# ylongqi/openrec

Hardware: AMD Instinct MI355X
Metric: BPR training triplets/sec at dim=64, 1Mx1M table (higher is better)
Workload: dtype f32; 1 GPU; bpr dim=64 1000000x1000000 table, batch=65536 triplets/GPU, sgd lr=0.05, objective loss+l2_loss, exact TF duplicate semantics; parallelism=single-gpu

## Files before the change

openrec_amd/csrc/kernels_plan.hip:

```cpp
#include "orx_internal.h"

#include "orx_device.h"

#include <cstring>
#include <vector>
#include <algorithm>

constexpr int PL_THREADS = 256;
constexpr int PL_REFS = 8;
constexpr int PL_CHUNK = PL_THREADS * PL_REFS;
constexpr int PL_LCNT = 1024;

struct PlanArgs {
    DedupArgs d;
    int shift;
    int nru, nri;
    int lgu, lgi;
    int* bcnt;
    int2* list;
    int64_t nref;
    unsigned int* dupbits;
    int min_late;
    int s_first;
    unsigned long long* tstamp;
};
#define PL_STAMP(i) do { if (a.tstamp != nullptr && threadIdx.x == 0) a.tstamp[((size_t)blockIdx.y * gridDim.x + blockIdx.x) * 8 + (i)] = wall_clock64(); } while (0)

__device__ __forceinline__ bool plan_ref(const PlanArgs& a, int64_t s, int64_t j, int& id, bool& is_user, int& pos) {
    const DedupArgs& d = a.d;
    if (j < d.nU) { id = d.uid[s * d.id_stride + j]; is_user = true; pos = (int)j; }
    else if (j < d.nU + d.nP) { id = d.pid[s * d.id_stride + (j - d.nU)]; is_user = false; pos = (int)(d.role_stride ? d.role_stride + (j - d.nU) : j); }
    else { id = d.nid[s * d.id_stride + (j - d.nU - d.nP)]; is_user = false; pos = (int)(d.role_stride ? 2 * d.role_stride + (j - d.nU - d.nP) : j); }
    return id_ok(id, is_user ? d.NU : d.NI);
}

__device__ __forceinline__ int32_t* plan_idword(const DedupArgs& d, int64_t s, int pos) {
    if (d.pair_tpw > 1) {
        const int Bp = (int)d.role_stride;
        const int slot = (pos >= Bp ? 1 : 0) + (pos >= 2 * Bp ? 1 : 0);
        return reinterpret_cast<int32_t*>(d.ids4 + s * d.pair_stride + (pos - slot * Bp)) + slot;
    }
    return d.ids_out + s * d.flag_stride + pos;
}

__device__ __forceinline__ void pl_lds_barrier() { asm volatile("s_waitcnt lgkmcnt(0)\n\ts_barrier" ::: "memory"); }

template <int T = PL_THREADS>
__device__ __forceinline__ int plan_scan_excl(int v, int* wave_tot, int& total) {
    const int lane = threadIdx.x & 63, wave = threadIdx.x >> 6;
    int incl = v;
#pragma unroll
    for (int o = 1; o < 64; o <<= 1) { const int t = __shfl_up(incl, o); if (lane >= o) incl += t; }
    if (lane == 63) wave_tot[wave] = incl;
    pl_lds_barrier();
    int before = 0, all = 0;
#pragma unroll
    for (int k = 0; k < T / 64; ++k) { const int t = wave_tot[k]; if (k < wave) before += t; all += t; }
    pl_lds_barrier();
    total = all;
    return before + incl - v;
}

template <bool SCATTER>
__global__ __launch_bounds__(PL_THREADS) void plan_part_kernel(PlanArgs a) {
    extern __shared__ int pl_hist[];
    const int nb = a.nru + a.nri;
    const int64_t s = blockIdx.y;
    int* hist = pl_hist;
    int* base = pl_hist + nb;
    for (int i = threadIdx.x; i < nb; i += PL_THREADS) hist[i] = 0;
    __syncthreads();
    const int64_t j0 = (int64_t)blockIdx.x * PL_CHUNK + threadIdx.x;
    int bk[PL_REFS], rk[PL_REFS], idv[PL_REFS], posv[PL_REFS];
#pragma unroll
    for (int k = 0; k < PL_REFS; ++k) {
        const int64_t j = j0 + (int64_t)k * PL_THREADS;
        bk[k] = -1;
        if (j < a.nref) {
            int id, pos; bool is_user;
            const bool ok = plan_ref(a, s, j, id, is_user, pos);
            if (ok) {
                bk[k] = is_user ? (id & (a.nru - 1)) : a.nru + (id & (a.nri - 1));
                idv[k] = id; posv[k] = pos;
            }
            if (SCATTER) {
                if (a.d.pair_tpw > 1) {
                    if (j < a.d.pair_stride) {
                        const int p = a.d.pid[s * a.d.id_stride + j];
                        const int n = a.d.label ? __float_as_int(a.d.label[s * a.d.id_stride + j]) : a.d.nid[s * a.d.id_stride + j];
                        const bool okp = id_ok(p, a.d.NI), okn = a.d.label ? true : id_ok(n, a.d.NI);
                        a.d.ids4[s * a.d.pair_stride + j] = make_int4(ok ? id : 0x7fffffff, okp ? p : 0x7fffffff, okn ? n : 0x7fffffff, (int)((uint32_t)j << 10));
                        if (!(ok & okp & okn)) {
                            const int poison = (int)(ORX_PARTNER_POISON | ((uint32_t)a.d.pair_gen << 24));
                            a.d.partner[s * a.d.pair_stride + j] = make_int4(poison, poison, poison, 0);
                        }
                    }
                } else {
                    a.d.ids_out[s * a.d.flag_stride + pos] = ok ? id : 0x7fffffff;
                }
            }
        }
    }
#pragma unroll
    for (int k = 0; k < PL_REFS; ++k) if (bk[k] >= 0) rk[k] = atomicAdd(&hist[bk[k]], 1);
    __syncthreads();
    int* cnt = a.bcnt + s * (3 * nb + 1);
    if (!SCATTER) {
        if (blockIdx.x == 0 && threadIdx.x < 8) a.d.alloc[8 * s + threadIdx.x] = 0;
        if (blockIdx.x == 0 && threadIdx.x == 8) a.d.dcount[s] = 0;
        for (int i = threadIdx.x; i < nb; i += PL_THREADS) { const int c = hist[i]; if (c) atomicAdd(cnt + i, c); }
        return;
    }
    __shared__ int wave_tot[PL_THREADS / 64];
    int* off = pl_hist + 2 * nb;
    for (int i = threadIdx.x; i < nb; i += PL_THREADS) off[i] = cnt[i];
    __syncthreads();
    {
        const int per = (nb + PL_THREADS - 1) / PL_THREADS;
        const int i0 = threadIdx.x * per;
        int mine = 0;
        for (int i = i0; i < i0 + per && i < nb; ++i) mine += off[i];
        int total;
        int run = plan_scan_excl(mine, wave_tot, total);
        for (int i = i0; i < i0 + per && i < nb; ++i) { const int c = off[i]; off[i] = run; run += c; }
        if (threadIdx.x == 0) off[nb] = total;
    }
    __syncthreads();
    if (blockIdx.x == 0) for (int i = threadIdx.x; i <= nb; i += PL_THREADS) cnt[2 * nb + i] = off[i];
    int* cur = cnt + nb;
    for (int i = threadIdx.x; i < nb; i += PL_THREADS) { const int c = hist[i]; if (c) base[i] = off[i] + atomicAdd(cur + i, c); }
    __syncthreads();
    int2* list = a.list + s * a.nref;
#pragma unroll
    for (int k = 0; k < PL_REFS; ++k) if (bk[k] >= 0) list[base[bk[k]] + rk[k]] = make_int2(idv[k], posv[k]);
}

__device__ __forceinline__ int pl_cnt(const int* p) { return __hip_atomic_load(p, __ATOMIC_RELAXED, __HIP_MEMORY_SCOPE_AGENT); }
__device__ __forceinline__ unsigned int pl_peek(const unsigned int* p) { return *reinterpret_cast<const volatile unsigned int*>(p); }

constexpr int PL_UN = 8;
template <int T, class F>
__device__ __forceinline__ void pl_for_each(const int2* ent, int n, F f) {
    for (int i0 = threadIdx.x; i0 < n; i0 += PL_UN * T) {
        int2 e[PL_UN];
#pragma unroll
        for (int k = 0; k < PL_UN; ++k) { const int i = i0 + k * T; if (i < n) e[k] = ent[i]; }
#pragma unroll
        for (int k = 0; k < PL_UN; ++k) { const int i = i0 + k * T; if (i < n) f(i, e[k]); }
    }
}

__device__ __forceinline__ int pl_rank(int* cnt, int dn) {
    const int lane = threadIdx.x & 63;
    int rank = -1;
    for (int round = 0; round < 4; ++round) {
        const unsigned long long todo = __ballot(rank < 0);
        if (!todo) break;
        const int ld = __shfl(dn, __ffsll((long long)todo) - 1);
        const bool mine = rank < 0 && dn == ld;
        const unsigned long long grp = __ballot(mine);
        const int gsz = __popcll(grp);
        if (gsz < 4) break;
        const int first = __ffsll((long long)grp) - 1;
        int base = 0;
        if (lane == first) base = atomicAdd(cnt + ld, gsz);
        base = __shfl(base, first);
        if (mine) rank = base + __popcll(grp & ((1ull << lane) - 1ull));
    }
    if (rank < 0) rank = atomicAdd(cnt + dn, 1);
    return rank;
}

constexpr int PL_PAIR_CAP = 512;

template <int T>
__global__ __launch_bounds__(T) void plan_range_kernel(PlanArgs a) {
    extern __shared__ __attribute__((aligned(16))) unsigned int pl_lds[];
    const DedupArgs& d = a.d;
    const int W = (1 << a.shift) >> 5;
    unsigned int* seen = pl_lds;
    unsigned int* dup = pl_lds + W;
    unsigned int* tri = pl_lds + 2 * W;
    unsigned short* prefix16 = reinterpret_cast<unsigned short*>(pl_lds + 3 * W);
    int* lcnt = reinterpret_cast<int*>(pl_lds + 3 * W + (W + 1) / 2);
    unsigned short* dprefix16 = reinterpret_cast<unsigned short*>(seen);
    int* pairpos = reinterpret_cast<int*>(lcnt + PL_LCNT);
    __shared__ int wave_tot[T / 64];
    __shared__ int sh_late, sh_dense, sh_seg, list_cnt, list_base;
    const int nb = a.nru + a.nri;
    const int b = blockIdx.x;
    const int64_t s = blockIdx.y;
    const bool is_user = b < a.nru;
    const int lg = is_user ? a.lgu : a.lgi;
    const int bl = is_user ? b : b - a.nru;
    const int* cnt = a.bcnt + s * (3 * nb + 1) + 2 * nb;
    PL_STAMP(0);
    if (b == 0) for (int i = threadIdx.x; i < 2 * nb; i += T) a.bcnt[s * (3 * nb + 1) + i] = 0;
    const int lo = cnt[b], n = cnt[b + 1] - lo;
    int2* ent = a.list + s * a.nref + lo;
    unsigned int* dupout = a.dupbits ? a.dupbits + ((size_t)s * nb + b) * W : nullptr;
    if (threadIdx.x == 0 && n > 8192) atomicMax(d.alloc + 8 * s + 6, n);
    if (n == 0) {
        if (dupout) for (int w = threadIdx.x; w < W; w += T) dupout[w] = 0u;
        return;
    }
    int2* refinfo = d.refinfo ? d.refinfo + s * d.flag_stride : nullptr;
    const bool small = n <= PL_UN * T;
    int2 er[PL_UN];
    if (small) {
#pragma unroll
        for (int k = 0; k < PL_UN; ++k) { const int i = threadIdx.x + k * T; if (i < n) er[k] = ent[i]; }
    }
    for (int i = threadIdx.x; i < 3 * W; i += T) pl_lds[i] = 0u;
    if (threadIdx.x == 0) { sh_late = 0; list_cnt = 0; }
    pl_lds_barrier();
    PL_STAMP(1);
    int late = 0;
    auto pass1 = [&](int2 e) -> int {
        const int l = e.x >> lg;
        const unsigned int bit = 1u << (l & 31);
        const unsigned int cur = pl_peek(&seen[l >> 5]);
        const unsigned int old = (cur & bit) ? cur : atomicOr(&seen[l >> 5], bit);
        int role = 0;
        if (old & bit) {
            const unsigned int cur2 = pl_peek(&dup[l >> 5]);
            const unsigned int old2 = (cur2 & bit) ? cur2 : atomicOr(&dup[l >> 5], bit);
            role = 1;
            if (old2 & bit) {
                if (!(pl_peek(&tri[l >> 5]) & bit)) atomicOr(&tri[l >> 5], bit);
                role = 2; ++late;
            }
        }
        return role;
    };
    if (small) {
#pragma unroll
        for (int k = 0; k < PL_UN; ++k) {
            const int i = threadIdx.x + k * T;
            if (i < n) er[k].y = (int)((uint32_t)er[k].y | ((uint32_t)pass1(er[k]) << 30));
        }
    } else {
        pl_for_each<T>(ent, n, [&](int i, int2 e) {
            const int role = pass1(e);
            if (role) ent[i].y = (int)((uint32_t)e.y | ((uint32_t)role << 30));
        });
    }
    if (late) atomicAdd(&sh_late, late);
    pl_lds_barrier();
    PL_STAMP(2);
    int mine = 0;
    for (int w = threadIdx.x; w < W; w += T) mine += __popc(dup[w]);
    int off = 0;
    if (mine) off = atomicAdd(&list_cnt, mine);
    pl_lds_barrier();
    int list_base_r = 0;
    if (threadIdx.x == 0 && list_cnt) {
        list_base_r = atomicAdd(d.dcount + s, list_cnt);
        atomicAdd(d.alloc + 8 * s + 5, list_cnt);
    }
    const bool want_plan = sh_late >= (a.min_late < 0 ? (n / 512 > 64 ? n / 512 : 64) : a.min_late);
    const bool plan = refinfo != nullptr && want_plan;
    if (want_plan && refinfo == nullptr && threadIdx.x == 0) atomicAdd(d.alloc + 8 * s + 1, sh_late);
    int ntri = 0, dense0 = 0;
    int* segstart = nullptr;
    if (plan) {
        segstart = d.segstart + s * d.tri_stride;
        const int per = (W + T - 1) / T;
        const int w0 = threadIdx.x * per;
        int mine3 = 0;
        for (int w = w0; w < w0 + per && w < W; ++w) mine3 += __popc(tri[w]);
        int pre = plan_scan_excl<T>(mine3, wave_tot, ntri);
        if (ntri > 65535) ntri = 0;
        if (ntri) {
            if (threadIdx.x == 0) sh_dense = atomicAdd(d.alloc + 8 * s, ntri);
            for (int w = w0; w < w0 + per && w < W; ++w) { prefix16[w] = (unsigned short)pre; pre += __popc(tri[w]); }
            __syncthreads();
            dense0 = sh_dense;
            if (ntri > PL_LCNT) lcnt = d.tricnt + s * d.tri_stride + dense0;
            for (int i = threadIdx.x; i < ntri; i += T) lcnt[i] = 0;
            __syncthreads();
        }
    }
    int ndup2 = 0;
    const bool pairing = d.pair_tpw > 1 && W <= 4096;
    if (pairing) {
        const int per = (W + T - 1) / T;
        const int w0 = threadIdx.x * per;
        int mine2 = 0;
        for (int w = w0; w < w0 + per && w < W; ++w) mine2 += __popc(dup[w] & ~tri[w]);
        int pre = plan_scan_excl<T>(mine2, wave_tot, ndup2);
        if (ndup2 > PL_PAIR_CAP) ndup2 = 0;
        if (ndup2) {
            for (int w = w0; w < w0 + per && w < W; ++w) { dprefix16[w] = (unsigned short)pre; pre += __popc(dup[w] & ~tri[w]); }
            for (int i = threadIdx.x; i < 2 * ndup2; i += T) pairpos[i] = -1;
            pl_lds_barrier();
        }
    }
    PL_STAMP(3);
    auto pass2 = [&](int2 e) {
        const int l = e.x >> lg;
        const int pos = e.y & 0x3fffffff;
        const unsigned int dw = dup[l >> 5];
        const unsigned int dd = (dw >> (l & 31)) & 1u;
        if (dd) {
            uint32_t v = (uint32_t)e.x | (1u << 31);
            const unsigned int tw = tri[l >> 5];
            const unsigned int t3 = (tw >> (l & 31)) & 1u;
            if (ndup2 && !t3) {
                const int dn2 = (int)dprefix16[l >> 5] + __popc(dw & ~tw & ((1u << (l & 31)) - 1u));
                pairpos[2 * dn2 + (int)(((uint32_t)e.y >> 30) & 1u)] = pos;
                return;
            }
            v |= (t3 ? 2u : ((uint32_t)e.y >> 30)) << 29;
            if (t3 && ntri) {
                const int dn = (int)prefix16[l >> 5] + __popc(tw & ((1u << (l & 31)) - 1u));
                refinfo[pos] = make_int2(dense0 + dn, pl_rank(lcnt, dn));
            } else if (t3 && refinfo != nullptr) {
                refinfo[pos] = make_int2(-1, 0);
            }
            *plan_idword(d, s, pos) = (int32_t)v;
        }
    };
    if (small) {
#pragma unroll
        for (int k = 0; k < PL_UN; ++k) { const int i = threadIdx.x + k * T; if (i < n) pass2(er[k]); }
    } else {
        pl_for_each<T>(ent, n, [&](int, int2 e) { pass2(e); });
    }
    PL_STAMP(4);
    if (ndup2) {
        pl_lds_barrier();
        int* partner = reinterpret_cast<int*>(d.partner + s * d.pair_stride);
        const int Bp = (int)d.role_stride;
        for (int k = threadIdx.x; k < ndup2; k += T) {
            const int posA = pairpos[2 * k], posB = pairpos[2 * k + 1];
            const int sa = (posA >= Bp ? 1 : 0) + (posA >= 2 * Bp ? 1 : 0), sb = (posB >= Bp ? 1 : 0) + (posB >= 2 * Bp ? 1 : 0);
            const int tag = d.pair_gen << 24;
            partner[4 * (posA - sa * Bp) + sa] = posB | tag;
            partner[4 * (posB - sb * Bp) + sb] = posA | (1 << 30) | tag;
        }
    }
    PL_STAMP(5);
    if (dupout) for (int w = threadIdx.x; w < W; w += T) dupout[w] = ndup2 ? tri[w] : dup[w];
    if (ntri) {
        __syncthreads();
        const int per = (ntri + T - 1) / T;
        const int d0 = threadIdx.x * per;
        int csum = 0;
        for (int k = d0; k < d0 + per && k < ntri; ++k) csum += pl_cnt(lcnt + k);
        int total_refs;
        int run = plan_scan_excl<T>(csum, wave_tot, total_refs);
        if (threadIdx.x == 0) sh_seg = atomicAdd(d.alloc + 8 * s + 1, total_refs);
        __syncthreads();
        run += sh_seg;
        for (int k = d0; k < d0 + per && k < ntri; ++k) { segstart[dense0 + k] = run; run += pl_cnt(lcnt + k); }
        __syncthreads();
    }
    PL_STAMP(6);
    if (threadIdx.x == 0) list_base = list_base_r;
    pl_lds_barrier();
    PL_STAMP(7);
    if (mine) {
        int64_t e = s * d.list_stride + list_base + off;
        const uint32_t tag = is_user ? 0u : 0x80000000u;
        for (int w = threadIdx.x; w < W; w += T) {
            unsigned int m = dup[w];
            const unsigned int m0 = m;
            const unsigned int tw = tri[w];
            while (m) {
                const int bpos = __ffs(m) - 1;
                m &= m - 1;
                if (ndup2 && !((tw >> bpos) & 1u)) {
                    const int dn2 = (int)dprefix16[w] + __popc(m0 & ~tw & ((1u << bpos) - 1u));
                    reinterpret_cast<int2*>(d.pslot)[e] = make_int2(pairpos[2 * dn2], pairpos[2 * dn2 + 1]);
                    if (d.dcnt != nullptr) { d.dseg[e] = 0; d.dcnt[e] = 0; }
                    ++e;
                    continue;
                }
                if (d.pair_tpw > 1) reinterpret_cast<int2*>(d.pslot)[e] = make_int2(-1, -1);
                d.dlist[e] = (uint32_t)((((int64_t)w * 32 + bpos) << lg) | bl) | tag;
                if (d.dcnt != nullptr) {
                    int c = 0, sg = 0;
                    if (ntri && ((tw >> bpos) & 1u)) {
                        const int dn = (int)prefix16[w] + __popc(tw & ((1u << bpos) - 1u));
                        c = pl_cnt(lcnt + dn);
                        sg = __hip_atomic_load(segstart + dense0 + dn, __ATOMIC_RELAXED, __HIP_MEMORY_SCOPE_AGENT);
                        if (c > ORX_SEG_DIRECT) {
                            int4* items = d.items + s * d.item_stride;
                            int src = sg, len = c, level = 0;
                            do {
                                const int pieces = (len + ORX_PIECE - 1) / ORX_PIECE;
                                const int b0 = d.tree_off[level] + atomicAdd(d.alloc + 8 * s + 2 + level, pieces);
                                for (int k = 0; k < pieces; ++k) {
                                    const int rem = len - k * ORX_PIECE;
                                    items[b0 + k] = make_int4(src + k * ORX_PIECE, rem < ORX_PIECE ? rem : ORX_PIECE, b0 + k, 0);
                                }
                                src = b0; len = pieces; ++level;
                            } while (len > ORX_SEG_DIRECT && level < 3);
                            sg = src; c = -len;
                        }
                    }
                    d.dseg[e] = sg; d.dcnt[e] = c;
                }
                ++e;
            }
        }
    }
}

template <int T>
__global__ __launch_bounds__(T) void plan_urgent_kernel(PlanArgs a) {
    extern __shared__ __attribute__((aligned(16))) unsigned int pl_lds[];
    const int W = (1 << a.shift) >> 5;
    const int nb = a.nru + a.nri;
    const int b = blockIdx.x;
    const int64_t s = a.s_first + blockIdx.y;
    const int* cnt = a.bcnt + s * (3 * nb + 1) + 2 * nb;
    const int lo = cnt[b], n = cnt[b + 1] - lo;
    if (n == 0) return;
    const int prev_n = cnt[b + 1 - (3 * nb + 1)] - cnt[b - (3 * nb + 1)];
    if (prev_n < 2) return;
    const unsigned int* prev = a.dupbits + ((s - 1) * nb + b) * (int64_t)W;
    for (int w = threadIdx.x; w < W; w += T) pl_lds[w] = prev[w];
    __syncthreads();
    const int lg = b < a.nru ? a.lgu : a.lgi;
    const int2* ent = a.list + s * a.nref + lo;
    pl_for_each<T>(ent, n, [&](int, int2 e) {
        const int l = e.x >> lg;
        if ((pl_lds[l >> 5] >> (l & 31)) & 1u) *plan_idword(a.d, s, e.y & 0x3fffffff) |= (1 << 28);
    });
}

__global__ __launch_bounds__(256) void plan_pair_kernel(PlanArgs a) {
    const DedupArgs& d = a.d;
    const int64_t s = blockIdx.y;
    const int B = (int)d.pair_stride, Bp = (int)d.role_stride, tpw = d.pair_tpw;
    const int4* part = d.partner + s * d.pair_stride;
    int* pword = reinterpret_cast<int*>(d.ids4 + s * d.pair_stride) + 3;
    const int nb = a.nru + a.nri, W = (1 << a.shift) >> 5;
    const int n = d.dcount[s];
    auto slot_of = [&](int pos) { return (pos >= Bp ? 1 : 0) + (pos >= 2 * Bp ? 1 : 0); };
    const uint32_t gen = (uint32_t)d.pair_gen;
    auto live = [gen](int w) { return (((uint32_t)w >> 24) & 63u) == gen && ((uint32_t)w & ORX_PARTNER_POS) != ORX_PARTNER_POISON; };
    auto poisoned = [gen](int4 r) {
        auto p = [gen](int w) { return (((uint32_t)w >> 24) & 63u) == gen && ((uint32_t)w & ORX_PARTNER_POS) == ORX_PARTNER_POISON; };
        return p(r.x) | p(r.y) | p(r.z);
    };
    auto choice = [live](int4 r) { return live(r.x) ? 0 : (live(r.y) ? 1 : (live(r.z) ? 2 : -1)); };
    auto word = [](int4 r, int k) { return k == 0 ? r.x : (k == 1 ? r.y : r.z); };
    const int4 none = make_int4(0, 0, 0, 0);
    int npair = 0;
    for (int e = blockIdx.x * 256 + threadIdx.x; e < n; e += gridDim.x * 256) {
        const int64_t eg = s * d.list_stride + e;
        const int2 ab = reinterpret_cast<const int2*>(d.pslot)[eg];
        const int posA = ab.x, posB = ab.y;
        if (posA < 0) continue;
        const int sa = slot_of(posA), sb = slot_of(posB);
        const int ta = posA - sa * Bp, tb = posB - sb * Bp;
        const int lo = ta < tb ? ta : tb, hi = ta < tb ? tb : ta;
        const int bl = lo ^ 1, bh = hi ^ 1;
        const bool same = (lo & ~(tpw - 1)) == (hi & ~(tpw - 1));
        const bool needq = ta != tb && !same;
        const int4 ra = part[ta], rb = part[tb];
        const int4 rl = (needq && bl < B) ? part[bl] : none, rh = (needq && bh < B) ? part[bh] : none;
        const bool mutual = (ta != tb) & (choice(ra) == sa) & (choice(rb) == sb) & !(poisoned(ra) | poisoned(rb));
        const int cl = choice(rl), ch = choice(rh);
        const int ppl = (int)((uint32_t)word(rl, cl) & ORX_PARTNER_POS), pph = (int)((uint32_t)word(rh, ch) & ORX_PARTNER_POS);
        const int syl = slot_of(ppl), syh = slot_of(pph);
        const int yl = ppl - syl * Bp, yh = pph - syh * Bp;
        const int4 ryl = (cl >= 0 && yl != bl) ? part[yl] : none, ryh = (ch >= 0 && yh != bh) ? part[yh] : none;
        const bool lo_taken = bl >= B || (cl >= 0 && yl != bl && choice(ryl) == syl);
        const bool hi_taken = bh >= B || (ch >= 0 && yh != bh && choice(ryh) == syh);
        bool acc = false;
        int stay = 0, mover = 0, q = 0;
        if (mutual) {
            if (same) { acc = true; stay = lo; mover = hi; q = hi; }
            else if (!lo_taken) { acc = true; stay = lo; mover = hi; q = bl; }
            else if (!hi_taken) { acc = true; stay = hi; mover = lo; q = bh; }
        }
        if (acc) {
            d.dlist[eg] = ORX_DLIST_DEAD;
            const uint32_t s_stay = (uint32_t)(stay == ta ? sa : sb), s_mov = (uint32_t)(stay == ta ? sb : sa), m = (uint32_t)tpw - 1u;
            pword[4 * stay] = (int)(ORX_PAIR_VALID | ORX_PAIR_WRITER | ((uint32_t)q & m) | (s_stay << 4) | (s_mov << 6) | ((uint32_t)stay << 10));
            pword[4 * q] = (int)(ORX_PAIR_VALID | ((uint32_t)stay & m) | (s_mov << 4) | (s_stay << 6) | ((uint32_t)mover << 10));
            if (q != mover) pword[4 * mover] = (int)((uint32_t)q << 10);
            reinterpret_cast<int2*>(d.pslot)[eg] = q != mover ? make_int2(q, mover) : make_int2(-1, -1);
            npair += 1;
        } else {
            reinterpret_cast<int2*>(d.pslot)[eg] = make_int2(-1, -1);
            int32_t* wa = plan_idword(d, s, posA);
            const uint32_t id = (uint32_t)*wa;
            *wa = (int32_t)(id | (1u << 31));
            *plan_idword(d, s, posB) = (int32_t)(id | (1u << 31) | (1u << 29));
            d.dlist[eg] = id | (sa ? 0x80000000u : 0u);
            if (a.dupbits != nullptr) {
                const int bk = sa ? a.nru + (int)(id & (uint32_t)(a.nri - 1)) : (int)(id & (uint32_t)(a.nru - 1));
                const int l = (int)(id >> (sa ? a.lgi : a.lgu));
                atomicOr(a.dupbits + ((size_t)s * nb + bk) * W + (l >> 5), 1u << (l & 31));
            }
        }
    }
    __shared__ int sh_np;
    if (threadIdx.x == 0) sh_np = 0;
    __syncthreads();
    if (npair) atomicAdd(&sh_np, npair);
    __syncthreads();
    if (threadIdx.x == 0 && sh_np) atomicAdd(d.alloc + 8 * s + 7, sh_np);
}

__global__ __launch_bounds__(256) void plan_swap_kernel(DedupArgs d) {
    const int64_t s = blockIdx.y;
    const int n = d.dcount[s];
    int4* rec = d.ids4 + s * d.pair_stride;
    for (int e = blockIdx.x * 256 + threadIdx.x; e < n; e += gridDim.x * 256) {
        const int2 qm = reinterpret_cast<const int2*>(d.pslot)[s * d.list_stride + e];
        if (qm.x < 0 || qm.y < 0) continue;
        const int4 a = rec[qm.x], b = rec[qm.y];
        rec[qm.x] = make_int4(b.x, b.y, b.z, a.w);
        rec[qm.y] = make_int4(a.x, a.y, a.z, b.w);
    }
}

int orx_launch_plan_swap(orx_ctx* ctx, const DedupArgs& d, int64_t kc) {
    if (d.pair_tpw < 2 || kc <= 0) return ORX_OK;
    ProfScope ps(ctx, ORX_K_DEDUP);
    ORX_LAUNCH(ctx, plan_swap_kernel, dim3((unsigned)std::max<int64_t>(4, (d.pair_stride / 4 + 255) / 256), (unsigned)kc), dim3(256), 0, d);
    ORX_HIP(hipGetLastError());
    return ORX_OK;
}

static int plan_buckets(int64_t rows, int64_t nref_t) {
    if (rows <= 0 || nref_t <= 0) return 0;
    const int cap = rows > (1LL << 27) ? 18 : 17;
    int64_t want = std::max<int64_t>((rows + (1LL << cap) - 1) >> cap, std::min<int64_t>(nref_t / 2048, rows / 64));
    static const char* env = getenv("ORX_PLAN_SHIFT");
    if (env) want = std::max<int64_t>(want, (rows + (1LL << atoi(env)) - 1) >> atoi(env));
    int n = 1;
    while (n < want && n < 8192) n *= 2;
    return n;
}
static int ilog2(int64_t n) { int l = 0; while ((1LL << l) < n) ++l; return l; }
static void plan_geometry(const DedupArgs& d, PlanArgs* a) {
    a->nref = d.nU + d.nP + d.nN;
    a->nru = plan_buckets(d.nU ? d.NU : 0, d.nU);
    a->nri = plan_buckets((d.nP + d.nN) ? d.NI : 0, d.nP + d.nN);
    a->lgu = ilog2(a->nru > 0 ? a->nru : 1); a->lgi = ilog2(a->nri > 0 ? a->nri : 1);
    const int64_t per_u = a->nru ? (d.NU + a->nru - 1) / a->nru : 1, per_i = a->nri ? (d.NI + a->nri - 1) / a->nri : 1;
    a->shift = std::max(5, ilog2(std::max(per_u, per_i)));
}

void orx_plan_geometry_query(const DedupArgs& d, int32_t out[14]) {
    PlanArgs a;
    plan_geometry(d, &a);
    out[0] = a.nru; out[1] = a.nri; out[2] = a.lgu; out[3] = a.lgi; out[4] = a.shift; out[5] = (1 << a.shift) >> 5;
    out[6] = PL_UN; out[7] = PL_LCNT; out[8] = PL_PAIR_CAP; out[9] = ORX_SEG_DIRECT; out[10] = ORX_PIECE;
    out[11] = PL_THREADS; out[12] = 1024; out[13] = PL_CHUNK;
}

static int plan_ensure(orx_ctx* c, int64_t chunk, const PlanArgs& a, bool want_dupbits) {
    const int nb = a.nru + a.nri;
    if (orx_ensure((void**)&c->d_pl_cnt, &c->d_pl_cnt_cap, (size_t)chunk * (3 * nb + 1) * sizeof(int))) return ORX_ERR_OOM;
    if (orx_ensure((void**)&c->d_pl_list, &c->d_pl_list_cap, (size_t)chunk * a.nref * sizeof(int2))) return ORX_ERR_OOM;
    const size_t words = (size_t)nb * ((1u << a.shift) >> 5);
    if (want_dupbits && orx_ensure((void**)&c->d_dupbits, &c->d_dupbits_cap, (size_t)chunk * words * sizeof(unsigned int))) return ORX_ERR_OOM;
    return ORX_OK;
}

int orx_plan_buffers(orx_ctx* c, int64_t chunk, int64_t B, int64_t NU, int64_t NI, bool want_dupbits) {
    const int64_t shapes[3][3] = {{B, B, B}, {B, B, 0}, {0, B, 0}};
    for (const auto& sh : shapes) {
        DedupArgs d;
        memset(&d, 0, sizeof(d));
        d.nU = sh[0]; d.nP = sh[1]; d.nN = sh[2]; d.NU = NU; d.NI = NI;
        PlanArgs a;
        plan_geometry(d, &a);
        const int rc = plan_ensure(c, chunk, a, want_dupbits);
        if (rc != ORX_OK) return rc;
    }
    return ORX_OK;
}

int orx_launch_plan(orx_ctx* ctx, const DedupArgs& d, int64_t kc, bool keep_dupbits, int64_t step0) {
    ProfScope ps(ctx, ORX_K_DEDUP);
    PlanArgs a;
    a.d = d;
    plan_geometry(d, &a);
    const int nb = a.nru + a.nri;
    if (nb == 0 || a.nref == 0 || kc == 0) return ORX_OK;
    ORX_ARG(a.nref < (1LL << 30) && kc < 65536, "plan: too many references per step (%lld) or steps (%lld)", (long long)a.nref, (long long)kc);
    { const int rc = plan_ensure(ctx, step0 + kc, a, keep_dupbits); if (rc != ORX_OK) return rc; }
    const size_t words = (size_t)nb * ((1u << a.shift) >> 5);
    a.bcnt = ctx->d_pl_cnt + step0 * (3 * nb + 1); a.list = ctx->d_pl_list + step0 * a.nref;
    a.dupbits = keep_dupbits ? ctx->d_dupbits + step0 * words : nullptr;
    a.s_first = 1;
    a.tstamp = nullptr;
    static const bool timing = getenv("ORX_PLAN_TIMING") != nullptr;
    if (timing) {
        ORX_HIP(hipMalloc((void**)&a.tstamp, (size_t)nb * kc * 8 * sizeof(unsigned long long)));
        ORX_HIP(hipMemsetAsync(a.tstamp, 0, (size_t)nb * kc * 8 * sizeof(unsigned long long), ctx->stream));
    }
    const char* ml = getenv("ORX_PLAN_MIN_LATE");
    a.min_late = ml ? atoi(ml) : d.min_late;
    if (ctx->pl_cnt_clean != ctx->d_pl_cnt || ctx->pl_cnt_clean_cap != ctx->d_pl_cnt_cap || ctx->pl_cnt_nb != nb)
        ORX_HIP(hipMemsetAsync(ctx->d_pl_cnt, 0, ctx->d_pl_cnt_cap, ctx->stream));
    ctx->pl_cnt_clean = nullptr;
    struct CleanMark { orx_ctx* c; int nb; bool ok = false;
                       ~CleanMark() { if (ok) { c->pl_cnt_clean = c->d_pl_cnt; c->pl_cnt_clean_cap = c->d_pl_cnt_cap; c->pl_cnt_nb = nb; } } } clean_mark{ctx, nb};
    const dim3 gp((unsigned)((a.nref + PL_CHUNK - 1) / PL_CHUNK), (unsigned)kc);
    const size_t hist_bytes = (size_t)(3 * nb + 1) * sizeof(int);
    ORX_ONCE_PER_DEVICE(ctx, ORX_HIP(hipFuncSetAttribute((const void*)plan_part_kernel<false>, hipFuncAttributeMaxDynamicSharedMemorySize, 128 * 1024)));
    ORX_ONCE_PER_DEVICE(ctx, ORX_HIP(hipFuncSetAttribute((const void*)plan_part_kernel<true>, hipFuncAttributeMaxDynamicSharedMemorySize, 128 * 1024)));
    ORX_ONCE_PER_DEVICE(ctx, ORX_HIP(hipFuncSetAttribute((const void*)plan_range_kernel<256>, hipFuncAttributeMaxDynamicSharedMemorySize, 140 * 1024)));
    ORX_ONCE_PER_DEVICE(ctx, ORX_HIP(hipFuncSetAttribute((const void*)plan_range_kernel<1024>, hipFuncAttributeMaxDynamicSharedMemorySize, 140 * 1024)));
    ORX_LAUNCH(ctx, (plan_part_kernel<false>), gp, dim3(PL_THREADS), hist_bytes, a);
    ORX_LAUNCH(ctx, (plan_part_kernel<true>), gp, dim3(PL_THREADS), hist_bytes, a);
    const int W = (1 << a.shift) >> 5;
    const size_t lds = (size_t)(3 * W + (W + 1) / 2) * 4 + (size_t)PL_LCNT * 4 +
                       (d.pair_tpw > 1 && W <= 4096 ? (size_t)2 * PL_PAIR_CAP * 4 : 0);
    if (ctx->plan_big) ORX_LAUNCH(ctx, plan_range_kernel<1024>, dim3((unsigned)nb, (unsigned)kc), dim3(1024), lds, a);
    else ORX_LAUNCH(ctx, plan_range_kernel<256>, dim3((unsigned)nb, (unsigned)kc), dim3(256), lds, a);
    if (d.pair_tpw > 1) ORX_LAUNCH(ctx, plan_pair_kernel, dim3((unsigned)std::max<int64_t>(4, (d.pair_stride / 4 + 255) / 256), (unsigned)kc), dim3(256), 0, a);
    ORX_HIP(hipGetLastError());
    clean_mark.ok = true;
    if (a.tstamp != nullptr) {
        ORX_HIP(hipStreamSynchronize(ctx->stream));
        std::vector<unsigned long long> h((size_t)nb * kc * 8);
        ORX_HIP(hipMemcpy(h.data(), a.tstamp, h.size() * sizeof(unsigned long long), hipMemcpyDeviceToHost));
        ORX_HIP(hipFree(a.tstamp));
        double sum[8] = {0}; unsigned long long t_min = ~0ull, t_max = 0; size_t live = 0;
        for (size_t w = 0; w < (size_t)nb * kc; ++w) {
            const unsigned long long* t = &h[w * 8];
            if (t[7] == 0) continue;
            ++live; t_min = std::min(t_min, t[0]); t_max = std::max(t_max, t[7]);
            for (int i = 1; i < 8; ++i) sum[i] += (double)(t[i] - t[i - 1]);
        }
        fprintf(stderr, "[orx plan timing] K=%lld, %zu workgroups, span %.1f us; mean us per phase: zero+cnt %.2f | pass1 %.2f | staging+prefix %.2f | pass2 %.2f | "
                "pairing %.2f | dupbits %.2f | list alloc %.2f\n", (long long)kc, live, (double)(t_max - t_min) * 0.01,
                sum[1] / live * 0.01, sum[2] / live * 0.01, sum[3] / live * 0.01, sum[4] / live * 0.01, sum[5] / live * 0.01, sum[6] / live * 0.01, sum[7] / live * 0.01);
    }
    return ORX_OK;
}

int orx_launch_plan_urgent(orx_ctx* ctx, const DedupArgs& d, int64_t kc, int64_t step0) {
    ProfScope ps(ctx, ORX_K_DEDUP);
    const int first = step0 > 0 ? 0 : 1;
    if (kc - first < 1) return ORX_OK;
    PlanArgs a;
    a.d = d;
    plan_geometry(d, &a);
    const int nb = a.nru + a.nri;
    const size_t words = (size_t)nb * ((1u << a.shift) >> 5);
    a.bcnt = ctx->d_pl_cnt + step0 * (3 * nb + 1); a.list = ctx->d_pl_list + step0 * a.nref; a.dupbits = ctx->d_dupbits + step0 * words; a.min_late = -1;
    a.s_first = first;
    a.tstamp = nullptr;
    const int W = (1 << a.shift) >> 5;
    if (ctx->plan_big) ORX_LAUNCH(ctx, plan_urgent_kernel<1024>, dim3((unsigned)(a.nru + a.nri), (unsigned)(kc - first)), dim3(1024), (size_t)W * 4, a);
    else ORX_LAUNCH(ctx, plan_urgent_kernel<256>, dim3((unsigned)(a.nru + a.nri), (unsigned)(kc - first)), dim3(256), (size_t)W * 4, a);
    ORX_HIP(hipGetLastError());
    return ORX_OK;
}
```

Baseline: 2.097 billion triplets/s.

## Flatten plan kernel grids and map each step's workgroups to one XCD

Replaces the 2D (block, step) launch grids of the plan kernels with a 1D grid. A remap function decodes each linear workgroup id so that all workgroups of a given step land on the same XCD under round-robin dispatch across the 8 XCDs. Per-step histogram atomics and count/list traffic then stay within one XCD's L2 instead of bouncing between XCDs. It adds index arithmetic per workgroup and depends on the hardware dispatching workgroups round-robin over XCDs.

```diff
diff --git a/openrec_amd/csrc/kernels_plan.hip b/openrec_amd/csrc/kernels_plan.hip
--- a/openrec_amd/csrc/kernels_plan.hip
+++ b/openrec_amd/csrc/kernels_plan.hip
@@ -1,6 +1,7 @@
 #include "orx_internal.h"
 
 #include "orx_device.h"
+#include "orx_plan_order.h"
 
 #include <cstring>
 #include <vector>
@@ -23,8 +24,10 @@
     int min_late;
     int s_first;
     unsigned long long* tstamp;
+    int gx, kc;
 };
-#define PL_STAMP(i) do { if (a.tstamp != nullptr && threadIdx.x == 0) a.tstamp[((size_t)blockIdx.y * gridDim.x + blockIdx.x) * 8 + (i)] = wall_clock64(); } while (0)
+#define PL_STAMP(i) do { if (a.tstamp != nullptr && threadIdx.x == 0) a.tstamp[((size_t)s * a.gx + b) * 8 + (i)] = wall_clock64(); } while (0)
+#define PL_WG(gx, kc) const OrxPlanWg pl_wg = orx_plan_order(blockIdx.x, (gx), (kc))
 
 __device__ __forceinline__ bool plan_ref(const PlanArgs& a, int64_t s, int64_t j, int& id, bool& is_user, int& pos) {
     const DedupArgs& d = a.d;
@@ -65,12 +68,14 @@
 __global__ __launch_bounds__(PL_THREADS) void plan_part_kernel(PlanArgs a) {
     extern __shared__ int pl_hist[];
     const int nb = a.nru + a.nri;
-    const int64_t s = blockIdx.y;
+    PL_WG(a.gx, a.kc);
+    const int64_t s = pl_wg.step;
+    const int blk = pl_wg.block;
     int* hist = pl_hist;
     int* base = pl_hist + nb;
     for (int i = threadIdx.x; i < nb; i += PL_THREADS) hist[i] = 0;
     __syncthreads();
-    const int64_t j0 = (int64_t)blockIdx.x * PL_CHUNK + threadIdx.x;
+    const int64_t j0 = (int64_t)blk * PL_CHUNK + threadIdx.x;
     int bk[PL_REFS], rk[PL_REFS], idv[PL_REFS], posv[PL_REFS];
 #pragma unroll
     for (int k = 0; k < PL_REFS; ++k) {
@@ -106,8 +111,8 @@
     __syncthreads();
     int* cnt = a.bcnt + s * (3 * nb + 1);
     if (!SCATTER) {
-        if (blockIdx.x == 0 && threadIdx.x < 8) a.d.alloc[8 * s + threadIdx.x] = 0;
-        if (blockIdx.x == 0 && threadIdx.x == 8) a.d.dcount[s] = 0;
+        if (blk == 0 && threadIdx.x < 8) a.d.alloc[8 * s + threadIdx.x] = 0;
+        if (blk == 0 && threadIdx.x == 8) a.d.dcount[s] = 0;
         for (int i = threadIdx.x; i < nb; i += PL_THREADS) { const int c = hist[i]; if (c) atomicAdd(cnt + i, c); }
         return;
     }
@@ -126,7 +131,7 @@
         if (threadIdx.x == 0) off[nb] = total;
     }
     __syncthreads();
-    if (blockIdx.x == 0) for (int i = threadIdx.x; i <= nb; i += PL_THREADS) cnt[2 * nb + i] = off[i];
+    if (blk == 0) for (int i = threadIdx.x; i <= nb; i += PL_THREADS) cnt[2 * nb + i] = off[i];
     int* cur = cnt + nb;
     for (int i = threadIdx.x; i < nb; i += PL_THREADS) { const int c = hist[i]; if (c) base[i] = off[i] + atomicAdd(cur + i, c); }
     __syncthreads();
@@ -188,8 +193,9 @@
     __shared__ int wave_tot[T / 64];
     __shared__ int sh_late, sh_dense, sh_seg, list_cnt, list_base;
     const int nb = a.nru + a.nri;
-    const int b = blockIdx.x;
-    const int64_t s = blockIdx.y;
+    PL_WG(a.gx, a.kc);
+    const int b = pl_wg.block;
+    const int64_t s = pl_wg.step;
     const bool is_user = b < a.nru;
     const int lg = is_user ? a.lgu : a.lgi;
     const int bl = is_user ? b : b - a.nru;
@@ -413,8 +419,9 @@
     extern __shared__ __attribute__((aligned(16))) unsigned int pl_lds[];
     const int W = (1 << a.shift) >> 5;
     const int nb = a.nru + a.nri;
-    const int b = blockIdx.x;
-    const int64_t s = a.s_first + blockIdx.y;
+    PL_WG(a.gx, a.kc);
+    const int b = pl_wg.block;
+    const int64_t s = a.s_first + pl_wg.step;
     const int* cnt = a.bcnt + s * (3 * nb + 1) + 2 * nb;
     const int lo = cnt[b], n = cnt[b + 1] - lo;
     if (n == 0) return;
@@ -433,7 +440,8 @@
 
 __global__ __launch_bounds__(256) void plan_pair_kernel(PlanArgs a) {
     const DedupArgs& d = a.d;
-    const int64_t s = blockIdx.y;
+    PL_WG(a.gx, a.kc);
+    const int64_t s = pl_wg.step;
     const int B = (int)d.pair_stride, Bp = (int)d.role_stride, tpw = d.pair_tpw;
     const int4* part = d.partner + s * d.pair_stride;
     int* pword = reinterpret_cast<int*>(d.ids4 + s * d.pair_stride) + 3;
@@ -450,7 +458,7 @@
     auto word = [](int4 r, int k) { return k == 0 ? r.x : (k == 1 ? r.y : r.z); };
     const int4 none = make_int4(0, 0, 0, 0);
     int npair = 0;
-    for (int e = blockIdx.x * 256 + threadIdx.x; e < n; e += gridDim.x * 256) {
+    for (int e = pl_wg.block * 256 + threadIdx.x; e < n; e += a.gx * 256) {
         const int64_t eg = s * d.list_stride + e;
         const int2 ab = reinterpret_cast<const int2*>(d.pslot)[eg];
         const int posA = ab.x, posB = ab.y;
@@ -508,11 +516,12 @@
     if (threadIdx.x == 0 && sh_np) atomicAdd(d.alloc + 8 * s + 7, sh_np);
 }
 
-__global__ __launch_bounds__(256) void plan_swap_kernel(DedupArgs d) {
-    const int64_t s = blockIdx.y;
+__global__ __launch_bounds__(256) void plan_swap_kernel(DedupArgs d, int gx, int kc) {
+    PL_WG(gx, kc);
+    const int64_t s = pl_wg.step;
     const int n = d.dcount[s];
     int4* rec = d.ids4 + s * d.pair_stride;
-    for (int e = blockIdx.x * 256 + threadIdx.x; e < n; e += gridDim.x * 256) {
+    for (int e = pl_wg.block * 256 + threadIdx.x; e < n; e += gx * 256) {
         const int2 qm = reinterpret_cast<const int2*>(d.pslot)[s * d.list_stride + e];
         if (qm.x < 0 || qm.y < 0) continue;
         const int4 a = rec[qm.x], b = rec[qm.y];
@@ -521,10 +530,15 @@
     }
 }
 
+static dim3 pl_grid(int64_t gx, int64_t kc) { return dim3((unsigned)(gx * kc)); }
+#define PL_GRID_OK(gx, kc) ORX_ARG((int64_t)(gx) * (int64_t)(kc) < (1LL << 31), "plan: %lld workgroups per step x %lld steps exceed a grid", (long long)(gx), (long long)(kc))
+
 int orx_launch_plan_swap(orx_ctx* ctx, const DedupArgs& d, int64_t kc) {
     if (d.pair_tpw < 2 || kc <= 0) return ORX_OK;
     ProfScope ps(ctx, ORX_K_DEDUP);
-    ORX_LAUNCH(ctx, plan_swap_kernel, dim3((unsigned)std::max<int64_t>(4, (d.pair_stride / 4 + 255) / 256), (unsigned)kc), dim3(256), 0, d);
+    const int gx = (int)std::max<int64_t>(4, (d.pair_stride / 4 + 255) / 256);
+    PL_GRID_OK(gx, kc);
+    ORX_LAUNCH(ctx, plan_swap_kernel, pl_grid(gx, kc), dim3(256), 0, d, gx, (int)kc);
     ORX_HIP(hipGetLastError());
     return ORX_OK;
 }
@@ -606,7 +620,10 @@
     ctx->pl_cnt_clean = nullptr;
     struct CleanMark { orx_ctx* c; int nb; bool ok = false;
                        ~CleanMark() { if (ok) { c->pl_cnt_clean = c->d_pl_cnt; c->pl_cnt_clean_cap = c->d_pl_cnt_cap; c->pl_cnt_nb = nb; } } } clean_mark{ctx, nb};
-    const dim3 gp((unsigned)((a.nref + PL_CHUNK - 1) / PL_CHUNK), (unsigned)kc);
+    a.kc = (int)kc;
+    a.gx = (int)((a.nref + PL_CHUNK - 1) / PL_CHUNK);
+    PL_GRID_OK(std::max<int64_t>(std::max(a.gx, nb), d.pair_stride / 1024 + 4), kc);
+    const dim3 gp = pl_grid(a.gx, kc);
     const size_t hist_bytes = (size_t)(3 * nb + 1) * sizeof(int);
     ORX_ONCE_PER_DEVICE(ctx, ORX_HIP(hipFuncSetAttribute((const void*)plan_part_kernel<false>, hipFuncAttributeMaxDynamicSharedMemorySize, 128 * 1024)));
     ORX_ONCE_PER_DEVICE(ctx, ORX_HIP(hipFuncSetAttribute((const void*)plan_part_kernel<true>, hipFuncAttributeMaxDynamicSharedMemorySize, 128 * 1024)));
@@ -617,9 +634,13 @@
     const int W = (1 << a.shift) >> 5;
     const size_t lds = (size_t)(3 * W + (W + 1) / 2) * 4 + (size_t)PL_LCNT * 4 +
                        (d.pair_tpw > 1 && W <= 4096 ? (size_t)2 * PL_PAIR_CAP * 4 : 0);
-    if (ctx->plan_big) ORX_LAUNCH(ctx, plan_range_kernel<1024>, dim3((unsigned)nb, (unsigned)kc), dim3(1024), lds, a);
-    else ORX_LAUNCH(ctx, plan_range_kernel<256>, dim3((unsigned)nb, (unsigned)kc), dim3(256), lds, a);
-    if (d.pair_tpw > 1) ORX_LAUNCH(ctx, plan_pair_kernel, dim3((unsigned)std::max<int64_t>(4, (d.pair_stride / 4 + 255) / 256), (unsigned)kc), dim3(256), 0, a);
+    a.gx = nb;
+    if (ctx->plan_big) ORX_LAUNCH(ctx, plan_range_kernel<1024>, pl_grid(nb, kc), dim3(1024), lds, a);
+    else ORX_LAUNCH(ctx, plan_range_kernel<256>, pl_grid(nb, kc), dim3(256), lds, a);
+    if (d.pair_tpw > 1) {
+        a.gx = (int)std::max<int64_t>(4, (d.pair_stride / 4 + 255) / 256);
+        ORX_LAUNCH(ctx, plan_pair_kernel, pl_grid(a.gx, kc), dim3(256), 0, a);
+    }
     ORX_HIP(hipGetLastError());
     clean_mark.ok = true;
     if (a.tstamp != nullptr) {
@@ -654,8 +675,10 @@
     a.s_first = first;
     a.tstamp = nullptr;
     const int W = (1 << a.shift) >> 5;
-    if (ctx->plan_big) ORX_LAUNCH(ctx, plan_urgent_kernel<1024>, dim3((unsigned)(a.nru + a.nri), (unsigned)(kc - first)), dim3(1024), (size_t)W * 4, a);
-    else ORX_LAUNCH(ctx, plan_urgent_kernel<256>, dim3((unsigned)(a.nru + a.nri), (unsigned)(kc - first)), dim3(256), (size_t)W * 4, a);
+    a.gx = nb; a.kc = (int)(kc - first);
+    PL_GRID_OK(nb, kc);
+    if (ctx->plan_big) ORX_LAUNCH(ctx, plan_urgent_kernel<1024>, pl_grid(nb, kc - first), dim3(1024), (size_t)W * 4, a);
+    else ORX_LAUNCH(ctx, plan_urgent_kernel<256>, pl_grid(nb, kc - first), dim3(256), (size_t)W * 4, a);
     ORX_HIP(hipGetLastError());
     return ORX_OK;
 }
diff --git a/openrec_amd/csrc/orx_plan_order.h b/openrec_amd/csrc/orx_plan_order.h
--- /dev/null
+++ b/openrec_amd/csrc/orx_plan_order.h
@@ -0,0 +1,25 @@
+#pragma once
+
+#ifndef ORX_HD
+#if defined(__HIPCC__) || defined(__CUDACC__)
+#define ORX_HD __host__ __device__
+#else
+#define ORX_HD
+#endif
+#endif
+
+struct OrxPlanWg { int step, block; };
+
+constexpr int ORX_PLAN_XCDS = 8;
+
+ORX_HD inline OrxPlanWg orx_plan_order(unsigned int L, int gx, int kc) {
+    const unsigned int per_group = (unsigned int)ORX_PLAN_XCDS * (unsigned int)gx;
+    const int g = (int)(L / per_group);
+    const unsigned int l = L - (unsigned int)g * per_group;
+    const int left = kc - g * ORX_PLAN_XCDS;
+    const unsigned int m = (unsigned int)(left < ORX_PLAN_XCDS ? left : ORX_PLAN_XCDS);
+    OrxPlanWg w;
+    w.step = g * ORX_PLAN_XCDS + (int)(l % m);
+    w.block = (int)(l / m);
+    return w;
+}
```

Result: faster. 2.135 billion triplets/s (median of 6 runs) (+1.8%).
